# tensor4all/tensor4all-rs

Hardware: AMD Instinct MI355X
Metric: TCI2 full-sweep GF/s (d=30, chi=256 fp64) (higher is better)
Workload: dtype f64

## Files before the change

### tensor4all-rs_amd/csrc/kernels.hpp

```cpp
#pragma once

#include <hip/hip_runtime.h>

#include <cstddef>
#include <cstdint>

#include "../../include/t4a_testfunctions.h"

namespace t4a {

struct RrluWorkspace;

struct RrluPlan {
    int W = 1;
    int T = 256;
    int cpw = 0;
    int Mld = 0;
    size_t lds_bytes = 0;
};

RrluPlan rrlu_make_plan(int M, int N, int num_cus);

struct RrluArgs {
    const double* A;
// ... 150 lines not shown
    unsigned long long* h_block;
    int block_u64;
    const int* dims;
    int dims_swap;
    const int* rowmap;
    XcdSpecArgs spec;
    int ts_u64;
};
bool rrlu_xcd_make_plan(int M, int N, RrluXcdPlan* out, bool any_size = false, int max_w = 32, bool allow_big = false);
size_t rrlu_xcd_keys_bytes(const RrluXcdPlan& plan);
size_t rrlu_xcd_cols_bytes(const RrluXcdPlan& plan, int M);
struct RrluXcdGroupArgs {
    RrluXcdArgs p[8];
};
void rrlu_xcd2_launch(const RrluXcdPlan& plan, const RrluXcdArgs& args, hipStream_t stream);
void rrlu_xcd2m_launch(const RrluXcdPlan& plan, const RrluXcdArgs& args, hipStream_t stream);
void rrlu_xcd2_group_launch(const RrluXcdPlan& plan, const RrluXcdGroupArgs& args, bool tie_row_major, hipStream_t stream);
bool rrlu_wg_make_plan(int M, int N, RrluXcdPlan* out, int spec_blocks = 0);
void rrlu_wg_launch(const RrluXcdPlan& plan, const RrluXcdArgs& args, hipStream_t stream);
void rrlu_wg_group_launch(const RrluXcdPlan& plan, const RrluXcdGroupArgs& args, bool tie_row_major, hipStream_t stream);
bool rrlu_w1_make_plan(int M, int N, RrluXcdPlan* out, int spec_blocks = 0);
void rrlu_w1_launch(const RrluXcdPlan& plan, const RrluXcdArgs& args, hipStream_t stream);
void rrlu_w1_group_launch(const RrluXcdPlan& plan, const RrluXcdGroupArgs& args, bool tie_row_major, hipStream_t stream);

void pi_eval_launch(const FnDevice& fn, const uint64_t* rowacc, int M, const uint64_t* colacc, int N, double* out,
                    int ld, bool transpose_out, unsigned long long* max_abs_bits, hipStream_t stream);
struct PiJob {
    const uint64_t* rowacc;
    const uint64_t* colacc;
    double* out;
    unsigned long long* max_abs_bits;
    int M, N, ld, pad_;
};
void pi_eval_batched_launch(const FnDevice& fn, const PiJob* d_jobs, int n_jobs, int max_M, int max_N, hipStream_t stream);
struct PackJob {
    const double* src;
    double* core;
    const int* info;
    int ld, L, S, R, last, pad_;
};
struct LuProblem;
constexpr int FILL_SMALL_MAX_N = 32, FILL_SMALL_MAX_RHS = 64;
void fill_small_launch(const FnDevice& fn, const PiJob* d_pis, const LuProblem* d_lups, const PackJob* d_packs, int n_jobs, int last_site,
                       hipStream_t stream);
void stage_copy_launch(const uint64_t* pinned_src, uint64_t* dst, size_t count, hipStream_t stream);
void absmax_launch(const double* data, size_t count, unsigned long long* max_abs_bits, hipStream_t stream);

constexpr int CHAIN_MAX_SET = 1024;
struct ChainTab {
    uint64_t* code;
    uint64_t* acc;
    int* cnt;
};
struct ChainCommon {
    ChainTab I, J, HI, HJ;
    ChainTab mI, mJ;
    int cap, K;
    const uint64_t* w;
    int total;
    const int* ldim;
    const int* woff;
    int forward, use_extras;
    int one_site;
    uint64_t* ind_code;
    uint64_t* ind_acc;
    int* ind_cnt;
    int ind_cap;
// ... 105 lines not shown
                               double* left, double* right, hipStream_t stream);
void transpose_launch(const double* in, int rows, int cols, int ldi, double* out, int ldo, hipStream_t stream);

struct TrsmProblem {
    const double* T; int ldt; int n;
    double* B; int ldb; int nrhs;
    int lower; int unit_diag;
    const int* skip_flag;
};
void trsm_left_batched_launch(const TrsmProblem* d_problems, int n_problems, int max_n, int max_nrhs, hipStream_t stream);

struct LuProblem {
    double* A; int lda; int n;
    int* piv;
    int* info;
    double* B; int ldb; int nrhs;
    const unsigned long long* pmax_bits;
};
void lu_batched_launch(const LuProblem* d_problems, int n_problems, int max_n, hipStream_t stream);
inline TrsmProblem lu_trsm_problem(const LuProblem& lp, bool lower, const int* skip_flag = nullptr)
{
    TrsmProblem t{};
    t.T = lp.A;
    t.ldt = lp.lda;
    t.n = lp.n;
    t.B = lp.B;
    t.ldb = lp.ldb;
    t.nrhs = lp.nrhs;
    t.lower = t.unit_diag = lower ? 1 : 0;
    t.skip_flag = skip_flag;
    return t;
}
constexpr int LU_MAX_PANEL_STEPS = 128;
bool lu_forward_blocked_launch(const LuProblem* d_problems, int n_problems, int max_n, int max_nrhs, hipStream_t stream, int avoid_xcc = -1,
                               unsigned* tickets = nullptr);
bool lu_solve_blocked_launch(const LuProblem* d_problems, int n_problems, int max_n, int max_nrhs, hipStream_t stream, int avoid_xcc = -1,
                             unsigned* tickets = nullptr);

void gather_launch(const double* in, int ldi, const int* rows, int nrows, const int* cols, int ncols, double* out,
                   int ldo, hipStream_t stream);
void scatter_rows_launch(const double* in, int ldi, const int* rows, int nrows, int ncols, double* out, int ldo,
                         hipStream_t stream);
void scatter_cols_launch(const double* in, int ldi, int nrows, const int* cols, int ncols, double* out, int ldo,
                         hipStream_t stream);
void fill_launch(double* p, size_t count, double value, hipStream_t stream);
void seq_matmul_launch(const double* A, int lda, const double* B, int ldb, double* C, int ldc, size_t M, size_t N, size_t K,
                       hipStream_t stream);
void set_identity_launch(double* p, int m, int n, int ld, hipStream_t stream);

struct TtCoreDesc { const double* data; int l, d, r; };
void tt_evaluate_launch(const TtCoreDesc* d_cores, int n_sites, int max_bond, const uint32_t* d_idx, int n_pts,
                        double* d_out, hipStream_t stream);


void core_reshape_launch(const double* in, int L, int S, int R, int mode, double* out, hipStream_t stream);
constexpr int PERMUTE_MAX_RANK = 16;
void permute_launch(const double* in, const size_t* dims, const size_t* perm, int rank, double* out, hipStream_t stream);
void tt_sum_launch(const TtCoreDesc* d_cores, int n_sites, int max_bond, double* d_out, hipStream_t stream);
void tt_norm2_step_launch(const TtCoreDesc& core, const double* d_cur, bool first, double* d_nxt, hipStream_t stream);
void tt_env_left_launch(const TtCoreDesc* d_cores, int split, int max_bond, const uint32_t* d_idx, int n_items,
                        double* d_out, int ld, hipStream_t stream);
void tt_env_right_launch(const TtCoreDesc* d_cores, int n_sites, int split, int max_bond, const uint32_t* d_idx,
                         int n_items, double* d_out, int ld, hipStream_t stream);
void tt_env_dot_launch(const double* d_left, const double* d_right, int len, int ld, const uint32_t* d_il,
                       const uint32_t* d_ir, size_t n_pts, double* d_out, hipStream_t stream);

struct MpoSiteJob {
    const double* A;
    const double* B;
// ... 100 lines not shown
```

### tensor4all-rs_amd/csrc/kernels_dense.hip

```cpp
#include "kernels.hpp"

#include <algorithm>
#include <atomic>
#include <map>
#include <mutex>
#include <utility>
#include "common.hpp"

#include <cstdlib>

namespace t4a {

namespace {

typedef double double4_t __attribute__((ext_vector_type(4)));

constexpr int GBM = 64, GBK = 32, GPAD = 4;

template <int BN>
__global__ void __launch_bounds__(256) gemm_kernel(GemmDesc d)
{
    extern __shared__ __attribute__((aligned(16))) char gemm_smem[];
    typedef double TileA[GBK][GBM + GPAD];
    typedef double TileB[GBK][BN + GPAD];
// ... 615 lines not shown
                for (int c = 0; c < NB; ++c) a[r][c] = U[c];
            }
            if (i == prow) {
#pragma unroll
                for (int c = 0; c < NB; ++c) a[r][c] = V[c];
            }
        }
    }
    const double piv = U[J];
    if (piv == 0.0 || piv != piv) return;
#pragma unroll
    for (int r = 0; r < RP; ++r) {
        const int i = tid + 256 * r;
        if (i > J && i < m) {
            const double l = a[r][J] / piv;
            a[r][J] = l;
#pragma unroll
            for (int c = J + 1; c < NB; ++c) {
                const double prod = l * U[c];
                a[r][c] = a[r][c] - prod;
            }
        }
    }
}

template <int NB, int RP, int... Js>
__device__ __forceinline__ void lu_panel_columns(double (&a)[RP][NB], const PanelShared& sh, const LuProblem& pr, int kb, int m, int w, int tid,
                                                 int& first_bad, std::integer_sequence<int, Js...>)
{
    (lu_panel_column<NB, RP, Js>(a, sh, pr, kb, m, w, tid, first_bad), ...);
}

template <int NB, int RP>
__global__ void __launch_bounds__(256) lu_panel_kernel(const LuProblem* problems, int kb)
{
    __shared__ double U[2 * NB], V[2 * NB];
    __shared__ double red_v[8];
    __shared__ int red_i[8];
    const LuProblem pr = problems[blockIdx.x];
    const int n = pr.n;
    const int tid = threadIdx.x;
    if (kb == 0) {
        if (pr.pmax_bits) {
            const double pmax = __longlong_as_double((long long)*pr.pmax_bits);
            if (pmax < 2.220446049250313e-16) {
                if (tid == 0) pr.info[0] = -1;
                return;
            }
        }
        if (tid == 0) pr.info[0] = 0;
    } else if (pr.info[0] == -1) {
        return;
    }
    if (kb >= n) return;
    const int m = n - kb, w = (n - kb) < NB ? (n - kb) : NB;
    double* A = pr.A;
    const int lda = pr.lda;
    double a[RP][NB];
#pragma unroll
    for (int r = 0; r < RP; ++r) {
        const int i = tid + 256 * r;
#pragma unroll
        for (int c = 0; c < NB; ++c) a[r][c] = (i < m && c < w) ? A[(size_t)(kb + c) * lda + kb + i] : 0.0;
    }
    int first_bad = 0;
    PanelShared sh{U, V, red_v, red_i};
    lu_panel_columns<NB, RP>(a, sh, pr, kb, m, w, tid, first_bad, std::make_integer_sequence<int, NB>{});
    if (tid == 0 && first_bad != 0 && pr.info[0] == 0) pr.info[0] = first_bad;
#pragma unroll
    for (int r = 0; r < RP; ++r) {
        const int i = tid + 256 * r;
#pragma unroll
        for (int c = 0; c < NB; ++c)
            if (i < m && c < w) A[(size_t)(kb + c) * lda + kb + i] = a[r][c];
    }
}

__global__ void __launch_bounds__(256) lu_update_kernel(const LuProblem* problems, int kb, int nb, int tiles, int n_problems, int avoid_xcc,
                                                        unsigned* ticket, int a_only)
{
    extern __shared__ __attribute__((aligned(16))) char smem_raw[];
    __shared__ int s_item;
    if (avoid_xcc >= 0) {
        unsigned xcc;
        asm volatile("s_getreg_b32 %0, hwreg(HW_REG_XCC_ID)" : "=s"(xcc));
        if ((int)(xcc & 0xF) == avoid_xcc) return;
    }
    const int total_items = tiles * n_problems;
    bool first = true;
    for (;;) {
    __syncthreads();
    if (threadIdx.x == 0) s_item = ticket ? (int)atomicAdd(ticket, 1u) : (first ? (int)blockIdx.x : total_items);
    __syncthreads();
    first = false;
    const int item = s_item;
    if (item >= total_items) break;
    const LuProblem pr = problems[item / tiles];
    const int n = pr.n;
    if (kb >= n || pr.info[0] == -1) continue;
    const int ta = (n + nb - 1) / nb;
    const int nrhs = pr.B ? pr.nrhs : 0;
    const int t = item % tiles;
    const bool in_a = t < ta;
    const int c0 = in_a ? t * nb : (t - ta) * nb;
    if (!in_a && (a_only || c0 >= nrhs)) continue;
    if (in_a && c0 == kb) continue;
    const int m = n - kb, w = (n - kb) < nb ? (n - kb) : nb;
    const int lim = in_a ? n : nrhs;
    const int tc = (lim - c0) < nb ? (lim - c0) : nb;
    const bool left = in_a && c0 < kb;
    const int tid = threadIdx.x, T = blockDim.x;
    const int ldp = m | 1;
    double* L = (double*)smem_raw;
    double* Tt = L + (size_t)ldp * nb;
    auto gcol = [&](int c) -> double* {
        return in_a ? pr.A + (size_t)(c0 + c) * pr.lda + kb : pr.B + (size_t)(c0 + c) * pr.ldb + kb;
    };
    {
        const double* const tbase = in_a ? pr.A + (size_t)c0 * pr.lda + kb : pr.B + (size_t)c0 * pr.ldb + kb;
// ... 85 lines not shown
        double* g = gcol(c);
        for (int i = tid; i < m; i += T) g[i] = Tt[(size_t)c * ldp + i];
    }
    }
}


constexpr int SVB = 16;
constexpr int SV_MAXS = 8;
template <int Q> __device__ __forceinline__ double quad_bcast_f64(double v)
{
    constexpr int ctrl = Q | (Q << 2) | (Q << 4) | (Q << 6);
    const long long b = __double_as_longlong(v);
    const int lo = __builtin_amdgcn_update_dpp(0, (int)(b & 0xFFFFFFFFll), ctrl, 0xF, 0xF, true);
    const int hi = __builtin_amdgcn_update_dpp(0, (int)(b >> 32), ctrl, 0xF, 0xF, true);
    return __longlong_as_double(((long long)hi << 32) | (unsigned int)lo);
}
template <int KK, bool LOWER> __device__ __forceinline__ void solve_block_step(double (&b)[4], const double (&dr)[SVB][4], const double (&rdr)[SVB], int g)
{
    constexpr int go = KK >> 2, to = KK & 3;
    double xk = quad_bcast_f64<go>(b[to]);
    if (!LOWER) xk = xk * rdr[KK];
    if (g == go) b[to] = xk;
#pragma unroll
    for (int t = 0; t < 4; ++t) b[t] = __builtin_fma(-dr[KK][t], xk, b[t]);
}
template <bool LOWER, int... KKs>
__device__ __forceinline__ void solve_block_steps(double (&b)[4], const double (&dr)[SVB][4], const double (&rdr)[SVB], int g, std::integer_sequence<int, KKs...>)
{
    if constexpr (LOWER) (solve_block_step<KKs, true>(b, dr, rdr, g), ...);
    else (solve_block_step<SVB - 1 - KKs, false>(b, dr, rdr, g), ...);
}

__global__ void __launch_bounds__(256) __attribute__((amdgpu_waves_per_eu(1, 1))) lu_solve_kernel(const LuProblem* problems, int cw, int n_problems, int chunks, int avoid_xcc, unsigned* ticket)
{
    extern __shared__ __attribute__((aligned(16))) char smem_raw[];
    __shared__ int s_item;
    if (avoid_xcc >= 0) {
        unsigned xcc;
        asm volatile("s_getreg_b32 %0, hwreg(HW_REG_XCC_ID)" : "=s"(xcc));
        if ((int)(xcc & 0xF) == avoid_xcc) return;
    }
    const int tid = threadIdx.x;
    const int lane = tid & 63, wave = tid >> 6;
    const int lr = lane & 15, lk = lane >> 4;
    const int cl = lane >> 2, g = lane & 3;
    const int total_items = chunks * n_problems;
    bool first = true;
    for (;;) {
        __syncthreads();
        if (tid == 0) s_item = ticket ? (int)atomicAdd(ticket, 1u) : (first ? (int)blockIdx.x : total_items);
        __syncthreads();
        first = false;
        const int item = s_item;
        if (item >= total_items) break;
        const LuProblem pr = problems[item / chunks];
        const int n = pr.n;
        const int c0 = (item % chunks) * cw;
        if (n <= 0 || !pr.B || c0 >= pr.nrhs || pr.info[0] == -1) continue;
        const int cwr = (pr.nrhs - c0) < cw ? (pr.nrhs - c0) : cw;
        const int ld = n | 1;
        double* Bs = reinterpret_cast<double*>(smem_raw);
        double* D = Bs + (size_t)ld * cw + ((ld * cw) & 1);
        double* rd = D + SVB * SVB;
        unsigned short* perm_s = reinterpret_cast<unsigned short*>(rd + SVB);
        unsigned short* piv_s = perm_s + ((n + 3) & ~3);
        typedef const double __attribute__((address_space(1)))* gcptr;
        typedef double __attribute__((address_space(1)))* gptr;
        const gcptr T = (gcptr)pr.A;
        const gptr Bg = (gptr)pr.B;
        const int ldt = pr.lda;
        {
            const int G = (n + 31) / 32;
            unsigned short* gs = reinterpret_cast<unsigned short*>(smem_raw);
// ... 401 lines not shown
            (void)hipFuncSetAttribute(reinterpret_cast<const void*>(&trsm_left_mfma_kernel), hipFuncAttributeMaxDynamicSharedMemorySize,
                                      160 * 1024);
            attr2 = true;
        }
        int cw = 32;
        const size_t per_col = (size_t)(max_n | 1) * 8;
        while (cw > 16 && (per_col * cw + (TRB + 1) * TRB * 8 > 150 * 1024 || (long long)n_problems * max_nrhs / cw < 1024)) cw -= 16;
        const size_t lds = per_col * cw + (size_t)(TRB + 1) * TRB * 8;
        if (lds <= 160 * 1024) {
            dim3 grid((max_nrhs + cw - 1) / cw, n_problems);
            hipLaunchKernelGGL(trsm_left_mfma_kernel, grid, dim3(256), lds, stream, d_problems, cw);
            return;
        }
    }
    int cw = (int)((128 * 1024) / ((size_t)max_n * 8));
    if (cw > 32) cw = 32;
    const long long total_cols = (long long)n_problems * max_nrhs;
    while (cw > 4 && total_cols / cw < 2048) cw /= 2;
    if (cw < 1) cw = 1;
    const size_t lds = (size_t)max_n * cw * 8;
    if (lds > 160 * 1024)
        throw Error(T4A_GPU_NOT_IMPLEMENTED, "triangular solve: systems with more than 20480 rows are not supported");
    dim3 grid((max_nrhs + cw - 1) / cw, n_problems);
    hipLaunchKernelGGL(trsm_left_kernel, grid, dim3(256), lds, stream, d_problems, cw);
}

void lu_batched_launch(const LuProblem* d_problems, int n_problems, int max_n, hipStream_t stream)
{
    if (n_problems <= 0) return;
    int T = max_n >= 128 ? 1024 : (max_n >= 32 ? 256 : 64);
    hipLaunchKernelGGL(lu_kernel, dim3(n_problems), dim3(T), 0, stream, d_problems);
}

bool lu_forward_blocked_launch(const LuProblem* d_problems, int n_problems, int max_n, int max_nrhs, hipStream_t stream, int avoid_xcc,
                               unsigned* tickets)
{
    if (n_problems <= 0 || max_n <= 0) return true;
    int nb;
    if (max_n <= 256) nb = 32;
    else if (max_n <= 512) nb = 16;
    else if (max_n <= 1024) nb = 8;
    else return false;
    static std::atomic<bool> attr_set{false};
    if (!attr_set) {
        (void)hipFuncSetAttribute(reinterpret_cast<const void*>(&lu_update_kernel),
                                  hipFuncAttributeMaxDynamicSharedMemorySize, 144 * 1024);
        (void)hipGetLastError();
        attr_set = true;
    }
    const int ldp = max_n | 1;
    const size_t lds_update = (size_t)ldp * nb * 8 * 2;
    const int tiles = (max_n + nb - 1) / nb + (max_nrhs + nb - 1) / nb + 1;
    for (int kb = 0; kb < max_n; kb += nb) {
        if (nb == 32) hipLaunchKernelGGL((lu_panel_kernel<32, 1>), dim3(n_problems), dim3(256), 0, stream, d_problems, kb);
        else if (nb == 16) hipLaunchKernelGGL((lu_panel_kernel<16, 2>), dim3(n_problems), dim3(256), 0, stream, d_problems, kb);
        else hipLaunchKernelGGL((lu_panel_kernel<8, 4>), dim3(n_problems), dim3(256), 0, stream, d_problems, kb);
        const int items = tiles * n_problems;
        unsigned* tk = tickets ? tickets + kb / nb : nullptr;
        const int grid = tk ? items + items / 7 + 8 : items;
        hipLaunchKernelGGL(lu_update_kernel, dim3(grid), dim3(256), lds_update, stream, d_problems, kb, nb, tiles, n_problems,
                           tk ? avoid_xcc : -1, tk, 0);
    }
    return true;
}

bool lu_solve_blocked_launch(const LuProblem* d_problems, int n_problems, int max_n, int max_nrhs, hipStream_t stream, int avoid_xcc,
                             unsigned* tickets)
{
    if (n_problems <= 0 || max_n <= 0) return true;
    if (max_n < 32 || max_n > 16 * 4 * SV_MAXS || max_nrhs < 16) return false;
    int nb;
    if (max_n <= 256) nb = 32;
    else nb = 16;
    static std::once_flag attr_once;
    std::call_once(attr_once, [] {
        (void)hipFuncSetAttribute(reinterpret_cast<const void*>(&lu_update_kernel), hipFuncAttributeMaxDynamicSharedMemorySize, 144 * 1024);
        (void)hipFuncSetAttribute(reinterpret_cast<const void*>(&lu_solve_kernel), hipFuncAttributeMaxDynamicSharedMemorySize, 160 * 1024);
        (void)hipGetLastError();
    });
    const int ldp = max_n | 1;
    const size_t lds_update = (size_t)ldp * nb * 8 * 2;
    const int tiles = (max_n + nb - 1) / nb;
    for (int kb = 0; kb < max_n; kb += nb) {
        if (nb == 32) hipLaunchKernelGGL((lu_panel_kernel<32, 1>), dim3(n_problems), dim3(256), 0, stream, d_problems, kb);
        else hipLaunchKernelGGL((lu_panel_kernel<16, 2>), dim3(n_problems), dim3(256), 0, stream, d_problems, kb);
        const int items = tiles * n_problems;
        unsigned* tk = tickets ? tickets + kb / nb : nullptr;
        const int grid = tk ? items + items / 7 + 8 : items;
        hipLaunchKernelGGL(lu_update_kernel, dim3(grid), dim3(256), lds_update, stream, d_problems, kb, nb, tiles, n_problems,
                           tk ? avoid_xcc : -1, tk, 1);
    }
    const size_t extra = (size_t)SVB * (SVB + 1) * 8 + SVB * 8 + 2 * (size_t)((max_n + 3) & ~3) * 2 + 64;
    int cw = 64;
    while (cw > 16 && (size_t)(max_n | 1) * cw * 8 + extra > 156 * 1024) cw -= 16;
    if (cw == 48) cw = 32;
    while (cw > 16 && max_nrhs <= cw / 2) cw /= 2;
    const size_t lds = (size_t)(max_n | 1) * cw * 8 + extra;
    const int chunks = (max_nrhs + cw - 1) / cw;
    const int items = chunks * n_problems;
    unsigned* tk = tickets ? tickets + (LU_MAX_PANEL_STEPS - 1) : nullptr;
    const int grid = tk ? items + items / 7 + 8 : items;
    hipLaunchKernelGGL(lu_solve_kernel, dim3(grid), dim3(256), lds, stream, d_problems, cw, n_problems, chunks, tk ? avoid_xcc : -1, tk);
    return true;
}

void tt_evaluate_launch(const TtCoreDesc* d_cores, int n_sites, int max_bond, const uint32_t* d_idx, int n_pts,
                        double* d_out, hipStream_t stream)
{
    if (n_pts <= 0) return;
    int blocks = n_pts < 4096 ? n_pts : 4096;
    const size_t lds = (size_t)2 * (max_bond > 0 ? max_bond : 1) * 8;
    hipLaunchKernelGGL(tt_eval_kernel, dim3(blocks), dim3(256), lds, stream, d_cores, n_sites, max_bond, d_idx, n_pts,
                       d_out);
}

}
```

### tensor4all-rs_amd/csrc/kernels_pi.hip

```cpp
#include "kernels.hpp"

namespace t4a {

namespace {

__device__ __forceinline__ void wave_absmax_commit(double av, unsigned long long* max_abs_bits)
{
#pragma unroll
    for (int off = 32; off >= 1; off >>= 1) {
        const double o = __shfl_xor(av, off);
        if (o > av) av = o;
    }
    if ((threadIdx.x & 63) == 0 && av > 0.0 && max_abs_bits)
        atomicMax(max_abs_bits, (unsigned long long)__double_as_longlong(av));
}

__global__ void __launch_bounds__(256) pi_eval_kernel(FnDevice fn, const uint64_t* __restrict__ rowacc, int M,
                                                      const uint64_t* __restrict__ colacc, int N,
                                                      double* __restrict__ out, int ld, int transpose_out,
                                                      unsigned long long* max_abs_bits)
{
    double av = 0.0;
    const int i = blockIdx.x * blockDim.x + threadIdx.x;
    uint64_t racc[T4A_FN_MAX_ACC] = {0, 0, 0, 0};
    if (i < M)
        for (int k = 0; k < fn.n_acc; ++k) racc[k] = rowacc[(size_t)i * fn.n_acc + k];
    for (int j = blockIdx.y; j < N; j += gridDim.y) {
        if (i < M) {
            uint64_t acc[T4A_FN_MAX_ACC] = {0, 0, 0, 0};
            for (int k = 0; k < fn.n_acc; ++k) acc[k] = racc[k] + colacc[(size_t)j * fn.n_acc + k];
            const double v = t4a_fn_value(fn.fid, acc, fn.params);
            if (transpose_out)
                out[(size_t)i * ld + j] = v;
            else
                out[(size_t)j * ld + i] = v;
            const double a = sqrt(v * v);
            if (a > av) av = a;
        }
    }
    wave_absmax_commit(av, max_abs_bits);
}

__global__ void __launch_bounds__(256) pi_eval_batched_kernel(FnDevice fn, const PiJob* __restrict__ jobs)
{
    const PiJob jb = jobs[blockIdx.z];
    double av = 0.0;
    const int i = blockIdx.x * blockDim.x + threadIdx.x;
    if (blockIdx.x * (int)blockDim.x >= jb.M) return;
    uint64_t racc[T4A_FN_MAX_ACC] = {0, 0, 0, 0};
    if (i < jb.M)
        for (int k = 0; k < fn.n_acc; ++k) racc[k] = jb.rowacc[(size_t)i * fn.n_acc + k];
    for (int j = blockIdx.y; j < jb.N; j += gridDim.y) {
        if (i < jb.M) {
            uint64_t acc[T4A_FN_MAX_ACC] = {0, 0, 0, 0};
            for (int k = 0; k < fn.n_acc; ++k) acc[k] = racc[k] + jb.colacc[(size_t)j * fn.n_acc + k];
            const double v = t4a_fn_value(fn.fid, acc, fn.params);
            jb.out[(size_t)j * jb.ld + i] = v;
            const double a = sqrt(v * v);
            if (a > av) av = a;
        }
    }
    wave_absmax_commit(av, jb.max_abs_bits);
}

__global__ void __launch_bounds__(256) absmax_kernel(const double* __restrict__ data, size_t count,
                                                     unsigned long long* max_abs_bits)
{
    double av = 0.0;
    for (size_t i = (size_t)blockIdx.x * blockDim.x + threadIdx.x; i < count; i += (size_t)gridDim.x * blockDim.x) {
        const double v = data[i];
        const double a = sqrt(v * v);
        if (a > av) av = a;
    }
    wave_absmax_commit(av, max_abs_bits);
}

__global__ void __launch_bounds__(256) stage_copy_kernel(const uint64_t* __restrict__ src, uint64_t* __restrict__ dst, size_t count)
{
    for (size_t i = (size_t)blockIdx.x * blockDim.x + threadIdx.x; i < count; i += (size_t)gridDim.x * blockDim.x) dst[i] = src[i];
}

}

void stage_copy_launch(const uint64_t* pinned_src, uint64_t* dst, size_t count, hipStream_t stream)
{
    if (count == 0) return;
    size_t blocks = (count + 255) / 256;
    if (blocks > 64) blocks = 64;
    hipLaunchKernelGGL(stage_copy_kernel, dim3((unsigned)blocks), dim3(256), 0, stream, pinned_src, dst, count);
}

void pi_eval_launch(const FnDevice& fn, const uint64_t* rowacc, int M, const uint64_t* colacc, int N, double* out,
                    int ld, bool transpose_out, unsigned long long* max_abs_bits, hipStream_t stream)
{
    if (M <= 0 || N <= 0) return;
    dim3 block(256);
    int gy = N < 2048 ? N : 2048;
    dim3 grid((M + 255) / 256, gy);
    hipLaunchKernelGGL(pi_eval_kernel, grid, block, 0, stream, fn, rowacc, M, colacc, N, out, ld,
                       transpose_out ? 1 : 0, max_abs_bits);
}

void pi_eval_batched_launch(const FnDevice& fn, const PiJob* d_jobs, int n_jobs, int max_M, int max_N, hipStream_t stream)
{
    if (n_jobs <= 0 || max_M <= 0 || max_N <= 0) return;
    const int gy = max_N < 512 ? max_N : 512;
    dim3 grid((max_M + 255) / 256, gy, n_jobs);
    hipLaunchKernelGGL(pi_eval_batched_kernel, grid, dim3(256), 0, stream, fn, d_jobs);
}

namespace {

struct FillSmallArgs {
    FnDevice fn;
    const PiJob* pis;
    const LuProblem* lups;
    const PackJob* packs;
    int n_jobs, last_site;
};

__global__ void __launch_bounds__(256) fill_small_kernel(FillSmallArgs a)
{
    __shared__ double As[FILL_SMALL_MAX_N * FILL_SMALL_MAX_N];
    __shared__ double Bs[FILL_SMALL_MAX_N * FILL_SMALL_MAX_RHS];
    __shared__ double red_v[4];
    __shared__ int red_i[4];
    __shared__ int piv_s, info_s;
    __shared__ double pivval_s;
    const int k = blockIdx.x, tid = threadIdx.x, T = blockDim.x, lane = tid & 63, wave = tid >> 6;
    if (k >= a.n_jobs) return;
    const bool last = a.last_site && k == a.n_jobs - 1;
    const int K = a.fn.n_acc;
    double pmax = 0.0;
    for (int q = 0; q < (last ? 1 : 2); ++q) {
        const PiJob jb = a.pis[2 * k + q];
        double* const dst = q == 0 ? Bs : As;
        double av = 0.0;
        for (int e = tid; e < jb.M * jb.N; e += T) {
            const int i = e % jb.M, j = e / jb.M;
            uint64_t acc[T4A_FN_MAX_ACC] = {0, 0, 0, 0};
            for (int c = 0; c < K; ++c) acc[c] = jb.rowacc[(size_t)i * K + c] + jb.colacc[(size_t)j * K + c];
// ... 156 lines not shown
```

### tensor4all-rs_amd/csrc/tci2.hip

```cpp
#include "tci2.hpp"

#include <thread>

#include <exception>

#include <algorithm>
#include <atomic>
#include <chrono>
#include <cmath>
#include <cstdlib>
#include <string>
#include <unordered_set>

namespace t4a {

extern thread_local double g_chain_wait_seconds;

namespace {

__global__ void __launch_bounds__(256) pack_left_core_kernel(const double* __restrict__ mat, int ldm, int mrows,
                                                             int mcols, double* __restrict__ core, int L, int S, int R)
{
    const size_t total = (size_t)L * S * R;
    for (size_t e = (size_t)blockIdx.x * blockDim.x + threadIdx.x; e < total; e += (size_t)gridDim.x * blockDim.x) {
// ... 914 lines not shown
    fill_last_sig_ = sig;
    ++fill_stats_[0];
    if (!done)
        for (auto& f : ops) f();
    if (fill_timed_) T4A_HIP(hipEventRecord(ev_fill_.b, st));
}

void Tci2::fill_wait()
{
    if (import_inflight_) {
        import_inflight_ = false;
        T4A_HIP(hipStreamSynchronize(import_stream_));
    }
    if (!fill_inflight_) return;
    fill_inflight_ = false;
    T4A_HIP(hipStreamSynchronize(fill_stream_));
    T4A_HIP(hipGetLastError());
    if (eng.prof.enabled && fill_timed_) {
        float ms = 0.f;
        T4A_HIP(hipEventElapsedTime(&ms, ev_fill_.a, ev_fill_.b));
        eng.prof.v[4] += ms;
        eng.prof.v[5] += 1.0;
    }
    fill_timed_ = false;
    for (size_t k = 0; k < fill_solved_sites_.size(); ++k)
        if (h_fillinfo_.get()[fill_solved_sites_[k]] > 0) {
            const size_t site = fill_solved_sites_[k];
            fill_solved_sites_.clear();
            throw Error(T4A_GPU_INTERNAL_ERROR, "one-site interpolation solve failed: singular pivot matrix at site " +
                                                    std::to_string(site));
        }
    fill_solved_sites_.clear();
}

void Tci2::fill_site_tensors_impl(bool async)
{
    fn_.require("tci2");
    const bool trust_cache = fill_cache_trusted_;
    fill_cache_trusted_ = false;
    static const bool host_prof_fill = std::getenv("T4A_HOST_PROFILE") != nullptr;
    const auto hpf_t0 = std::chrono::steady_clock::now();
    static double hpf_sec[10] = {0, 0, 0, 0, 0, 0, 0, 0, 0, 0};
    auto hpf_mark = [&](int k, std::chrono::steady_clock::time_point& t) {
        if (!host_prof_fill) return;
        const auto now = std::chrono::steady_clock::now();
        hpf_sec[k] += std::chrono::duration<double, std::micro>(now - t).count();
        t = now;
    };
    auto hpf_t = hpf_t0;
    if (!trust_cache) invalidate_fill_cache();
    if (!fn_.builtin()) sync_digits();
    fill_wait();
    if (!fill_stream_) fill_stream_ = pool::stream_get(2);
    const bool builtin = fn_.builtin();
    static const bool sync_fill = std::getenv("T4A_SYNC_FILL") != nullptr;
    if (!builtin || sync_fill) async = false;
    std::vector<std::function<void()>> ops;
    std::vector<uint64_t> sig;
    auto dev = [&](std::function<void()> f) { ops.push_back(std::move(f)); };
    auto sg = [&](uint64_t v) { sig.push_back(v); };
    const bool no_main_sync = fill_no_main_sync_ && fn_.builtin();
    fill_no_main_sync_ = false;
    if (!no_main_sync) T4A_HIP(hipStreamSynchronize(eng.stream()));
    hipStream_t st = fill_stream_;
    struct SiteJob {
        size_t b;
// ... 25 lines not shown
                dev([=]() { fill_launch(ptr, cnt, 0.0, st); });
            }
            continue;
        }
        SiteJob j;
        j.b = b;
        j.ni = ni;
        j.nj = nj;
        j.last = (b == n_ - 1);
        j.np = j.last ? 0 : i_set[b + 1].count;
        if (!j.last && j.np != nj)
            throw Error(T4A_GPU_INTERNAL_ERROR, "one-site interpolation solve failed: pivot matrix at bond " +
                                                    std::to_string(b) + " is not square (" + std::to_string(j.np) + " x " +
                                                    std::to_string(nj) + ")");
        j.offA = totA;
        j.offB = totB;
        j.accJ = j.accK = j.accI = 0;
        totA += j.last ? 0 : nj * j.np;
        totB += nj * ni;
        jobs.push_back(j);
    }
    hpf_mark(0, hpf_t);
    if (jobs.empty()) {
        for (auto& f : ops) f();
        T4A_HIP(hipStreamSynchronize(st));
        return;
    }
    if (!builtin) {
        for (auto& f : ops) f();
        ops.clear();
    }
    d_fillA_.reserve(std::max<size_t>(totA, 1));
    d_fillB_.reserve(totB);
    const size_t fm_words = n_ + (n_ + 1) / 2 + (LU_MAX_PANEL_STEPS + 1) / 2;
    d_fillmax_.reserve(fm_words);
    unsigned long long* d_max = d_fillmax_.get();
    int* d_info = reinterpret_cast<int*>(d_fillmax_.get() + n_);
    unsigned* d_tickets = reinterpret_cast<unsigned*>(d_fillmax_.get() + n_ + (n_ + 1) / 2);
    const int avoid_xcc = (no_main_sync && !xcd_disabled()) ? eng.xcc() : -1;
    h_fillinfo_.reserve(n_);
    {
        unsigned long long* ptr = d_fillmax_.get();
        const size_t bytes = fm_words * sizeof(unsigned long long);
        fill_timed_ = eng.prof.enabled;
        sg((uint64_t)(uintptr_t)ptr);
        sg((uint64_t)bytes);
        dev([=]() { T4A_HIP(hipMemsetAsync(ptr, 0, bytes, st)); });
        if (!builtin) {
            if (fill_timed_) T4A_HIP(hipEventRecord(ev_fill_.a, st));
            for (auto& f : ops) f();
            ops.clear();
            T4A_HIP(hipStreamSynchronize(st));
        }
    }

    for (const SiteJob& j : jobs) {
        const size_t left_dim = (j.b == 0) ? 1 : i_set[j.b].count;
        const size_t S = local_dims[j.b];
        DevCore& c = cores[j.b];
        c.l = left_dim;
        c.s = S;
        c.r = j.last ? 1 : j.np;
        c.buf.reserve(std::max<size_t>(c.size(), 1));
    }

    std::vector<LuProblem> lups;
    std::vector<TrsmProblem> trl, tru;
    std::vector<PackJob> packs;
    size_t piv_total = 0;
    for (const SiteJob& j : jobs)
        if (!j.last) piv_total += j.np;
    d_fillpiv_.reserve(std::max<size_t>(piv_total, 1));
// ... 115 lines not shown
                q.out = d_fillA_.get() + j.offA;
                q.max_abs_bits = d_max + j.b;
                pis.push_back(q);
            }
        }
        for (const PiJob& q : pis) {
            max_M = std::max(max_M, q.M);
            max_N = std::max(max_N, q.N);
        }
        std::memcpy(hb + off_pi, pis.data(), pis.size() * sizeof(PiJob));
        if (np_) {
            std::memcpy(hb + off_lu, lups.data(), bytes_lu);
            std::memcpy(hb + off_tr, trl.data(), np_ * sizeof(TrsmProblem));
            std::memcpy(hb + off_tr + np_ * sizeof(TrsmProblem), tru.data(), np_ * sizeof(TrsmProblem));
        }
        std::memcpy(hb + off_pk, packs.data(), bytes_pk);
        hpf_mark(7, hpf_t);
        {
            const FnDevice fn = fn_.dev;
            const PiJob* dj = reinterpret_cast<const PiJob*>(db + off_pi);
            const int npi = (int)pis.size();
            sg((uint64_t)(uintptr_t)db);
            sg((uint64_t)(uintptr_t)hb);
            sg((uint64_t)total_bytes);
            sg((uint64_t)npi);
            sg(((uint64_t)(uint32_t)max_M << 32) | (uint32_t)max_N);
            sg((uint64_t)fn.fid * 16 + (uint64_t)fn.n_acc);
            for (int q = 0; q < T4A_FN_MAX_PARAMS; ++q) {
                uint64_t bits;
                std::memcpy(&bits, &fn.params[q], sizeof(bits));
                sg(bits);
            }
            sg((uint64_t)small_fill);
            const bool small = small_fill;
            dev([=]() {
                T4A_HIP(hipMemcpyAsync(db, hb, total_bytes, hipMemcpyHostToDevice, st));
                if (!small) pi_eval_batched_launch(fn, dj, npi, max_M, max_N, st);
            });
        }
        d_lups = reinterpret_cast<const LuProblem*>(db + off_lu);
        d_trs = reinterpret_cast<const TrsmProblem*>(db + off_tr);
        d_packs = reinterpret_cast<const PackJob*>(db + off_pk);
        d_pis = reinterpret_cast<const PiJob*>(db + off_pi);
    } else {
        for (const SiteJob& j : jobs) {
            IndexSet ik = kronecker_i(j.b);
            const IndexSet& jb = j_set[j.b];
            if (j.last) {
                eval_matrix(ik, 0, jb, ik.width, d_fillB_.get() + j.offB, nullptr);
            } else {
                eval_matrix(jb, j.b + 1, ik, 0, d_fillB_.get() + j.offB, nullptr);
                eval_matrix(jb, j.b + 1, i_set[j.b + 1], 0, d_fillA_.get() + j.offA, d_max + j.b);
            }
        }
        T4A_HIP(hipStreamSynchronize(eng.stream()));
        acc_used_ = 0;
        const size_t off_tr = up8(bytes_lu), off_pk = up8(off_tr + bytes_tr), total_bytes = up8(off_pk + bytes_pk);
        h_fillacc_.reserve(total_bytes / 8 + 1);
        d_fillacc_.reserve(total_bytes / 8 + 1);
        char* hb = reinterpret_cast<char*>(h_fillacc_.get());
        char* db = reinterpret_cast<char*>(d_fillacc_.get());
        if (np_) {
            std::memcpy(hb, lups.data(), bytes_lu);
            std::memcpy(hb + off_tr, trl.data(), np_ * sizeof(TrsmProblem));
            std::memcpy(hb + off_tr + np_ * sizeof(TrsmProblem), tru.data(), np_ * sizeof(TrsmProblem));
        }
        std::memcpy(hb + off_pk, packs.data(), bytes_pk);
        T4A_HIP(hipMemcpyAsync(db, hb, total_bytes, hipMemcpyHostToDevice, st));
        d_lups = reinterpret_cast<const LuProblem*>(db);
        d_trs = reinterpret_cast<const TrsmProblem*>(db + off_tr);
        d_packs = reinterpret_cast<const PackJob*>(db + off_pk);
    }

    {
        const int npr = (int)np_;
        const unsigned gx = blocks_for(max_core) > 64 ? 64 : blocks_for(max_core), gy = (unsigned)packs.size();
        int* hinfo = h_fillinfo_.get();
        const size_t info_bytes = n_ * sizeof(int);
        sg((uint64_t)npr);
        sg((uint64_t)(int64_t)avoid_xcc);
        sg(((uint64_t)(uint32_t)max_n << 32) | (uint32_t)max_nrhs);
        sg(((uint64_t)gx << 32) | gy);
        sg((uint64_t)(uintptr_t)d_lups);
        sg((uint64_t)(uintptr_t)d_trs);
        sg((uint64_t)(uintptr_t)d_packs);
        sg((uint64_t)(uintptr_t)d_info);
        sg((uint64_t)(uintptr_t)hinfo);
        const FnDevice fn = fn_.dev;
        const int n_site_jobs = (int)jobs.size(), last_site = jobs.back().last ? 1 : 0;
        const bool small = small_fill;
        sg((uint64_t)(uintptr_t)d_pis);
        sg(((uint64_t)n_site_jobs << 1) | (uint64_t)last_site);
        dev([=]() {
            if (small) {
                fill_small_launch(fn, d_pis, d_lups, d_packs, n_site_jobs, last_site, st);
                T4A_HIP(hipMemcpyAsync(hinfo, d_info, info_bytes, hipMemcpyDeviceToHost, st));
                return;
            }
            if (npr) {
                if (!lu_solve_blocked_launch(d_lups, npr, max_n, max_nrhs, st, avoid_xcc, d_tickets)) {
                    if (!lu_forward_blocked_launch(d_lups, npr, max_n, max_nrhs, st, avoid_xcc, d_tickets)) {
                        lu_batched_launch(d_lups, npr, max_n, st);
                        trsm_left_batched_launch(d_trs, npr, max_n, max_nrhs, st);
                    }
                    trsm_left_batched_launch(d_trs + npr, npr, max_n, max_nrhs, st);
                }
            }
            hipLaunchKernelGGL(pack_fill_batched_kernel, dim3(gx, gy), dim3(256), 0, st, d_packs);
            T4A_HIP(hipMemcpyAsync(hinfo, d_info, info_bytes, hipMemcpyDeviceToHost, st));
        });
    }
    hpf_mark(3, hpf_t);
    eng.prof.v[10] += flops;
    if (!builtin) {
        for (auto& f : ops) f();
        if (fill_timed_) T4A_HIP(hipEventRecord(ev_fill_.b, st));
        fill_inflight_ = true;
    } else {
        issue_fill_ops(ops, sig);
        fill_inflight_ = true;
    }
    if (host_prof_fill) {
        static double acc_ms = 0;
        static long calls = 0;
        acc_ms += std::chrono::duration<double, std::milli>(std::chrono::steady_clock::now() - hpf_t0).count();
        hpf_mark(4, hpf_t);
        if (++calls % 20 == 0)
            std::fprintf(stderr, "[host profile] fill_site_tensors host part %.1f us per call (wait+jobs %.1f, descriptors %.1f, "
                                 "accumulators %.1f, staging %.1f, issue %.1f)\n",
                         1e3 * acc_ms / calls, hpf_sec[0] / calls, hpf_sec[1] / calls, hpf_sec[2] / calls, hpf_sec[3] / calls,
                         hpf_sec[4] / calls);
        if (calls % 20 == 0)
            std::fprintf(stderr, "[host profile]   staging in detail: reserve %.1f, accumulator copy %.1f, job tables %.1f us per call\n",
                         hpf_sec[5] / calls, hpf_sec[6] / calls, hpf_sec[7] / calls);
// ... 253 lines not shown
    r.small_complete = false;
    if (small_engine_run(r) && r.small_complete) return;
    if (fn_.builtin() && options.max_bond_dim != 0 && options.max_bond_dim <= 1024) {
        const size_t chi = options.max_bond_dim;
        std::vector<size_t> lb(n_ + 1, 1), rb(n_ + 1, 1);
        for (size_t b = 0; b < n_; ++b) lb[b + 1] = std::min(chi, lb[b] * local_dims[b]);
        for (size_t b = n_; b-- > 0;) rb[b] = std::min(chi, rb[b + 1] * local_dims[b]);
        auto bond = [&](size_t b) { return std::min(lb[b], rb[b]); };
        size_t totA = 0, totB = 0, tot_cores = 0;
        for (size_t b = 0; b < n_; ++b) {
            if (shard_world > 1 && (b % shard_world) != shard_rank) continue;
            const size_t l = bond(b), rr = bond(b + 1);
            tot_cores += l * local_dims[b] * rr;
            totA += rr * rr;
            totB += rr * l * local_dims[b];
        }
        const bool presize = (tot_cores + totA + totB) * sizeof(double) <= ((size_t)1 << 30);
        for (size_t b = 0; presize && b < n_; ++b) {
            if (shard_world > 1 && (b % shard_world) != shard_rank) continue;
            cores[b].buf.reserve(std::max<size_t>(bond(b) * local_dims[b] * bond(b + 1), 1));
        }
        if (presize) {
        d_fillA_.reserve(std::max<size_t>(totA, 1));
        d_fillB_.reserve(std::max<size_t>(totB, 1));
        d_fillpiv_.reserve(std::max<size_t>(n_ * chi, 1));
        size_t acc_words = 0;
        for (size_t b = 0; b < n_; ++b) {
            if (shard_world > 1 && (b % shard_world) != shard_rank) continue;
            acc_words += chi * (2 + local_dims[b]) * (size_t)fn_.dev.n_acc;
        }
        const size_t desc_bytes = n_ * (2 * sizeof(PiJob) + sizeof(LuProblem) + 2 * sizeof(TrsmProblem) + 64) + 256;
        h_fillacc_.reserve(acc_words + desc_bytes / 8 + 64);
        d_fillacc_.reserve(acc_words + desc_bytes / 8 + 64);
        d_fillmax_.reserve(n_ + (n_ + 1) / 2 + (LU_MAX_PANEL_STEPS + 1) / 2);
        h_fillinfo_.reserve(n_);
        }
    }
}

bool Tci2::opt_iter_start(OptRun& r, bool defer_launch)
{
    const TCI2Options& options = r.options;
    if (r.done || r.iter >= options.max_iter) return false;
    const size_t iter = r.iter;
    (void)iter;
        r.norm = (options.normalize_error && max_sample_value > 0.0) ? max_sample_value : 1.0;
        r.abs_tol = options.tolerance * r.norm;
        bool is_forward = true;
        if (options.sweep_strategy == 1) is_forward = false;
        else if (options.sweep_strategy == 2) is_forward = (iter % 2 == 0);

        long ext_idx = (!options.strictly_nested && !history.empty()) ? (long)history.size() - 1 : -1;
        {
            OptSeg seg_(0);
            HistEntry cur;
            cur.serial = ++chain_.hist_serial;
            if (chain_.digits_stale) {
                cur.digits_valid = false;
                cur.cap = chain_.cap;
                cur.is.resize(n_);
                cur.js.resize(n_);
                for (size_t p = 0; p < n_; ++p) {
                    cur.is[p].width = i_set[p].width;
                    cur.is[p].count = i_set[p].count;
                    cur.js[p].width = j_set[p].width;
                    cur.js[p].count = j_set[p].count;
                }
// ... 296 lines not shown
```

Measured before the change: 306.5.

## Steer fill kernels away from all XCDs busy with concurrent multi-XCD rrLU

```diff
diff --git a/tensor4all-rs_amd/csrc/kernels.hpp b/tensor4all-rs_amd/csrc/kernels.hpp
--- a/tensor4all-rs_amd/csrc/kernels.hpp
+++ b/tensor4all-rs_amd/csrc/kernels.hpp
@@ -206,7 +206,9 @@
     unsigned long long* max_abs_bits;
     int M, N, ld, pad_;
 };
-void pi_eval_batched_launch(const FnDevice& fn, const PiJob* d_jobs, int n_jobs, int max_M, int max_N, hipStream_t stream);
+constexpr int PI_MAX_ITEMS = 4096;
+void pi_eval_batched_launch(const FnDevice& fn, const PiJob* d_jobs, int n_jobs, int max_M, int max_N, hipStream_t stream,
+                            unsigned avoid_mask = 0, unsigned* ticket = nullptr);
 struct PackJob {
     const double* src;
     double* core;
@@ -378,9 +380,10 @@
     return t;
 }
 constexpr int LU_MAX_PANEL_STEPS = 128;
-bool lu_forward_blocked_launch(const LuProblem* d_problems, int n_problems, int max_n, int max_nrhs, hipStream_t stream, int avoid_xcc = -1,
+constexpr int LU_TICKET_WORDS = 2 * LU_MAX_PANEL_STEPS;
+bool lu_forward_blocked_launch(const LuProblem* d_problems, int n_problems, int max_n, int max_nrhs, hipStream_t stream, unsigned avoid_mask = 0,
                                unsigned* tickets = nullptr);
-bool lu_solve_blocked_launch(const LuProblem* d_problems, int n_problems, int max_n, int max_nrhs, hipStream_t stream, int avoid_xcc = -1,
+bool lu_solve_blocked_launch(const LuProblem* d_problems, int n_problems, int max_n, int max_nrhs, hipStream_t stream, unsigned avoid_mask = 0,
                              unsigned* tickets = nullptr);
 
 void gather_launch(const double* in, int ldi, const int* rows, int nrows, const int* cols, int ncols, double* out,
diff --git a/tensor4all-rs_amd/csrc/kernels_dense.hip b/tensor4all-rs_amd/csrc/kernels_dense.hip
--- a/tensor4all-rs_amd/csrc/kernels_dense.hip
+++ b/tensor4all-rs_amd/csrc/kernels_dense.hip
@@ -671,12 +671,8 @@
 }
 
 template <int NB, int RP>
-__global__ void __launch_bounds__(256) lu_panel_kernel(const LuProblem* problems, int kb)
-{
-    __shared__ double U[2 * NB], V[2 * NB];
-    __shared__ double red_v[8];
-    __shared__ int red_i[8];
-    const LuProblem pr = problems[blockIdx.x];
+__device__ __forceinline__ void lu_panel_problem(const LuProblem& pr, int kb, const PanelShared& sh)
+{
     const int n = pr.n;
     const int tid = threadIdx.x;
     if (kb == 0) {
@@ -703,7 +699,6 @@
         for (int c = 0; c < NB; ++c) a[r][c] = (i < m && c < w) ? A[(size_t)(kb + c) * lda + kb + i] : 0.0;
     }
     int first_bad = 0;
-    PanelShared sh{U, V, red_v, red_i};
     lu_panel_columns<NB, RP>(a, sh, pr, kb, m, w, tid, first_bad, std::make_integer_sequence<int, NB>{});
     if (tid == 0 && first_bad != 0 && pr.info[0] == 0) pr.info[0] = first_bad;
 #pragma unroll
@@ -715,15 +710,42 @@
     }
 }
 
-__global__ void __launch_bounds__(256) lu_update_kernel(const LuProblem* problems, int kb, int nb, int tiles, int n_problems, int avoid_xcc,
+template <int NB, int RP>
+__global__ void __launch_bounds__(256) __attribute__((amdgpu_waves_per_eu(5))) lu_panel_kernel(const LuProblem* problems, int kb, int n_problems, unsigned avoid_mask, unsigned* ticket)
+{
+    __shared__ double U[2 * NB], V[2 * NB];
+    __shared__ double red_v[8];
+    __shared__ int red_i[8];
+    __shared__ int s_item;
+    PanelShared sh{U, V, red_v, red_i};
+    if (!ticket) {
+        lu_panel_problem<NB, RP>(problems[blockIdx.x], kb, sh);
+        return;
+    }
+    {
+        unsigned xcc;
+        asm volatile("s_getreg_b32 %0, hwreg(HW_REG_XCC_ID)" : "=s"(xcc));
+        if ((avoid_mask >> (xcc & 0xF)) & 1u) return;
+    }
+    for (;;) {
+        __syncthreads();
+        if (threadIdx.x == 0) s_item = (int)atomicAdd(ticket, 1u);
+        __syncthreads();
+        const int item = __builtin_amdgcn_readfirstlane(s_item);
+        if (item >= n_problems) break;
+        lu_panel_problem<NB, RP>(problems[item], kb, sh);
+    }
+}
+
+__global__ void __launch_bounds__(256) lu_update_kernel(const LuProblem* problems, int kb, int nb, int tiles, int n_problems, unsigned avoid_mask,
                                                         unsigned* ticket, int a_only)
 {
     extern __shared__ __attribute__((aligned(16))) char smem_raw[];
     __shared__ int s_item;
-    if (avoid_xcc >= 0) {
+    if (avoid_mask) {
         unsigned xcc;
         asm volatile("s_getreg_b32 %0, hwreg(HW_REG_XCC_ID)" : "=s"(xcc));
-        if ((int)(xcc & 0xF) == avoid_xcc) return;
+        if ((avoid_mask >> (xcc & 0xF)) & 1u) return;
     }
     const int total_items = tiles * n_problems;
     bool first = true;
@@ -875,14 +897,14 @@
     else (solve_block_step<SVB - 1 - KKs, false>(b, dr, rdr, g), ...);
 }
 
-__global__ void __launch_bounds__(256) __attribute__((amdgpu_waves_per_eu(1, 1))) lu_solve_kernel(const LuProblem* problems, int cw, int n_problems, int chunks, int avoid_xcc, unsigned* ticket)
+__global__ void __launch_bounds__(256) __attribute__((amdgpu_waves_per_eu(1, 1))) lu_solve_kernel(const LuProblem* problems, int cw, int n_problems, int chunks, unsigned avoid_mask, unsigned* ticket)
 {
     extern __shared__ __attribute__((aligned(16))) char smem_raw[];
     __shared__ int s_item;
-    if (avoid_xcc >= 0) {
+    if (avoid_mask) {
         unsigned xcc;
         asm volatile("s_getreg_b32 %0, hwreg(HW_REG_XCC_ID)" : "=s"(xcc));
-        if ((int)(xcc & 0xF) == avoid_xcc) return;
+        if ((avoid_mask >> (xcc & 0xF)) & 1u) return;
     }
     const int tid = threadIdx.x;
     const int lane = tid & 63, wave = tid >> 6;
@@ -1350,7 +1372,7 @@
     hipLaunchKernelGGL(lu_kernel, dim3(n_problems), dim3(T), 0, stream, d_problems);
 }
 
-bool lu_forward_blocked_launch(const LuProblem* d_problems, int n_problems, int max_n, int max_nrhs, hipStream_t stream, int avoid_xcc,
+bool lu_forward_blocked_launch(const LuProblem* d_problems, int n_problems, int max_n, int max_nrhs, hipStream_t stream, unsigned avoid_mask,
                                unsigned* tickets)
 {
     if (n_problems <= 0 || max_n <= 0) return true;
@@ -1370,19 +1392,21 @@
     const size_t lds_update = (size_t)ldp * nb * 8 * 2;
     const int tiles = (max_n + nb - 1) / nb + (max_nrhs + nb - 1) / nb + 1;
     for (int kb = 0; kb < max_n; kb += nb) {
-        if (nb == 32) hipLaunchKernelGGL((lu_panel_kernel<32, 1>), dim3(n_problems), dim3(256), 0, stream, d_problems, kb);
-        else if (nb == 16) hipLaunchKernelGGL((lu_panel_kernel<16, 2>), dim3(n_problems), dim3(256), 0, stream, d_problems, kb);
-        else hipLaunchKernelGGL((lu_panel_kernel<8, 4>), dim3(n_problems), dim3(256), 0, stream, d_problems, kb);
+        unsigned* ptk = (tickets && avoid_mask) ? tickets + LU_MAX_PANEL_STEPS + kb / nb : nullptr;
+        const int pgrid = ptk ? n_problems + n_problems / 7 + 8 : n_problems;
+        if (nb == 32) hipLaunchKernelGGL((lu_panel_kernel<32, 1>), dim3(pgrid), dim3(256), 0, stream, d_problems, kb, n_problems, avoid_mask, ptk);
+        else if (nb == 16) hipLaunchKernelGGL((lu_panel_kernel<16, 2>), dim3(pgrid), dim3(256), 0, stream, d_problems, kb, n_problems, avoid_mask, ptk);
+        else hipLaunchKernelGGL((lu_panel_kernel<8, 4>), dim3(pgrid), dim3(256), 0, stream, d_problems, kb, n_problems, avoid_mask, ptk);
         const int items = tiles * n_problems;
         unsigned* tk = tickets ? tickets + kb / nb : nullptr;
         const int grid = tk ? items + items / 7 + 8 : items;
         hipLaunchKernelGGL(lu_update_kernel, dim3(grid), dim3(256), lds_update, stream, d_problems, kb, nb, tiles, n_problems,
-                           tk ? avoid_xcc : -1, tk, 0);
+                           tk ? avoid_mask : 0u, tk, 0);
     }
     return true;
 }
 
-bool lu_solve_blocked_launch(const LuProblem* d_problems, int n_problems, int max_n, int max_nrhs, hipStream_t stream, int avoid_xcc,
+bool lu_solve_blocked_launch(const LuProblem* d_problems, int n_problems, int max_n, int max_nrhs, hipStream_t stream, unsigned avoid_mask,
                              unsigned* tickets)
 {
     if (n_problems <= 0 || max_n <= 0) return true;
@@ -1400,13 +1424,15 @@
     const size_t lds_update = (size_t)ldp * nb * 8 * 2;
     const int tiles = (max_n + nb - 1) / nb;
     for (int kb = 0; kb < max_n; kb += nb) {
-        if (nb == 32) hipLaunchKernelGGL((lu_panel_kernel<32, 1>), dim3(n_problems), dim3(256), 0, stream, d_problems, kb);
-        else hipLaunchKernelGGL((lu_panel_kernel<16, 2>), dim3(n_problems), dim3(256), 0, stream, d_problems, kb);
+        unsigned* ptk = (tickets && avoid_mask) ? tickets + LU_MAX_PANEL_STEPS + kb / nb : nullptr;
+        const int pgrid = ptk ? n_problems + n_problems / 7 + 8 : n_problems;
+        if (nb == 32) hipLaunchKernelGGL((lu_panel_kernel<32, 1>), dim3(pgrid), dim3(256), 0, stream, d_problems, kb, n_problems, avoid_mask, ptk);
+        else hipLaunchKernelGGL((lu_panel_kernel<16, 2>), dim3(pgrid), dim3(256), 0, stream, d_problems, kb, n_problems, avoid_mask, ptk);
         const int items = tiles * n_problems;
         unsigned* tk = tickets ? tickets + kb / nb : nullptr;
         const int grid = tk ? items + items / 7 + 8 : items;
         hipLaunchKernelGGL(lu_update_kernel, dim3(grid), dim3(256), lds_update, stream, d_problems, kb, nb, tiles, n_problems,
-                           tk ? avoid_xcc : -1, tk, 1);
+                           tk ? avoid_mask : 0u, tk, 1);
     }
     const size_t extra = (size_t)SVB * (SVB + 1) * 8 + SVB * 8 + 2 * (size_t)((max_n + 3) & ~3) * 2 + 64;
     int cw = 64;
@@ -1418,7 +1444,7 @@
     const int items = chunks * n_problems;
     unsigned* tk = tickets ? tickets + (LU_MAX_PANEL_STEPS - 1) : nullptr;
     const int grid = tk ? items + items / 7 + 8 : items;
-    hipLaunchKernelGGL(lu_solve_kernel, dim3(grid), dim3(256), lds, stream, d_problems, cw, n_problems, chunks, tk ? avoid_xcc : -1, tk);
+    hipLaunchKernelGGL(lu_solve_kernel, dim3(grid), dim3(256), lds, stream, d_problems, cw, n_problems, chunks, tk ? avoid_mask : 0u, tk);
     return true;
 }
 
diff --git a/tensor4all-rs_amd/csrc/kernels_pi.hip b/tensor4all-rs_amd/csrc/kernels_pi.hip
--- a/tensor4all-rs_amd/csrc/kernels_pi.hip
+++ b/tensor4all-rs_amd/csrc/kernels_pi.hip
@@ -41,16 +41,14 @@
     wave_absmax_commit(av, max_abs_bits);
 }
 
-__global__ void __launch_bounds__(256) pi_eval_batched_kernel(FnDevice fn, const PiJob* __restrict__ jobs)
-{
-    const PiJob jb = jobs[blockIdx.z];
+__device__ __forceinline__ void pi_eval_job_columns(const FnDevice& fn, const PiJob& jb, int row0, int j0, int j1, int jstep)
+{
     double av = 0.0;
-    const int i = blockIdx.x * blockDim.x + threadIdx.x;
-    if (blockIdx.x * (int)blockDim.x >= jb.M) return;
+    const int i = row0 + (int)threadIdx.x;
     uint64_t racc[T4A_FN_MAX_ACC] = {0, 0, 0, 0};
     if (i < jb.M)
         for (int k = 0; k < fn.n_acc; ++k) racc[k] = jb.rowacc[(size_t)i * fn.n_acc + k];
-    for (int j = blockIdx.y; j < jb.N; j += gridDim.y) {
+    for (int j = j0; j < j1; j += jstep) {
         if (i < jb.M) {
             uint64_t acc[T4A_FN_MAX_ACC] = {0, 0, 0, 0};
             for (int k = 0; k < fn.n_acc; ++k) acc[k] = racc[k] + jb.colacc[(size_t)j * fn.n_acc + k];
@@ -63,6 +61,39 @@
     wave_absmax_commit(av, jb.max_abs_bits);
 }
 
+__global__ void __launch_bounds__(256) pi_eval_batched_kernel(FnDevice fn, const PiJob* __restrict__ jobs, unsigned avoid_mask,
+                                                              unsigned* ticket, int row_tiles, int col_blocks, int col_block, int n_jobs)
+{
+    if (!ticket) {
+        const PiJob jb = jobs[blockIdx.z];
+        if (blockIdx.x * (int)blockDim.x >= jb.M) return;
+        pi_eval_job_columns(fn, jb, blockIdx.x * blockDim.x, blockIdx.y, jb.N, gridDim.y);
+        return;
+    }
+    __shared__ int s_item;
+    {
+        unsigned xcc;
+        asm volatile("s_getreg_b32 %0, hwreg(HW_REG_XCC_ID)" : "=s"(xcc));
+        if ((avoid_mask >> (xcc & 0xF)) & 1u) return;
+    }
+    const int per_job = row_tiles * col_blocks, total_items = per_job * n_jobs;
+    if (threadIdx.x == 0) s_item = (int)atomicAdd(ticket, 1u);
+    __syncthreads();
+    int item = __builtin_amdgcn_readfirstlane(s_item);
+    while (item < total_items) {
+        unsigned next = 0;
+        if (threadIdx.x == 0) next = atomicAdd(ticket, 1u);
+        const PiJob jb = jobs[item / per_job];
+        const int r = item % per_job;
+        const int row0 = (r / col_blocks) * 256, c0 = (r % col_blocks) * col_block;
+        if (row0 < jb.M && c0 < jb.N) pi_eval_job_columns(fn, jb, row0, c0, (c0 + col_block) < jb.N ? (c0 + col_block) : jb.N, 1);
+        __syncthreads();
+        if (threadIdx.x == 0) s_item = (int)next;
+        __syncthreads();
+        item = __builtin_amdgcn_readfirstlane(s_item);
+    }
+}
+
 __global__ void __launch_bounds__(256) absmax_kernel(const double* __restrict__ data, size_t count,
                                                      unsigned long long* max_abs_bits)
 {
@@ -101,12 +132,23 @@
                        transpose_out ? 1 : 0, max_abs_bits);
 }
 
-void pi_eval_batched_launch(const FnDevice& fn, const PiJob* d_jobs, int n_jobs, int max_M, int max_N, hipStream_t stream)
+void pi_eval_batched_launch(const FnDevice& fn, const PiJob* d_jobs, int n_jobs, int max_M, int max_N, hipStream_t stream,
+                            unsigned avoid_mask, unsigned* ticket)
 {
     if (n_jobs <= 0 || max_M <= 0 || max_N <= 0) return;
+    const int row_tiles = (max_M + 255) / 256;
+    if (avoid_mask && ticket) {
+        int col_block = 4;
+        while ((long long)n_jobs * row_tiles * ((max_N + col_block - 1) / col_block) > PI_MAX_ITEMS) col_block *= 2;
+        const int col_blocks = (max_N + col_block - 1) / col_block;
+        const int items = n_jobs * row_tiles * col_blocks;
+        hipLaunchKernelGGL(pi_eval_batched_kernel, dim3(items + items / 7 + 8), dim3(256), 0, stream, fn, d_jobs, avoid_mask, ticket,
+                           row_tiles, col_blocks, col_block, n_jobs);
+        return;
+    }
     const int gy = max_N < 512 ? max_N : 512;
-    dim3 grid((max_M + 255) / 256, gy, n_jobs);
-    hipLaunchKernelGGL(pi_eval_batched_kernel, grid, dim3(256), 0, stream, fn, d_jobs);
+    dim3 grid(row_tiles, gy, n_jobs);
+    hipLaunchKernelGGL(pi_eval_batched_kernel, grid, dim3(256), 0, stream, fn, d_jobs, 0u, (unsigned*)nullptr, 0, 0, 0, n_jobs);
 }
 
 namespace {
diff --git a/tensor4all-rs_amd/csrc/tci2.hip b/tensor4all-rs_amd/csrc/tci2.hip
--- a/tensor4all-rs_amd/csrc/tci2.hip
+++ b/tensor4all-rs_amd/csrc/tci2.hip
@@ -970,6 +970,8 @@
         }
     fill_solved_sites_.clear();
 }
+
+static size_t fill_scratch_words(size_t n) { return n + (n + 1) / 2 + (LU_TICKET_WORDS + 1 + 1) / 2; }
 
 void Tci2::fill_site_tensors_impl(bool async)
 {
@@ -1061,12 +1063,20 @@
     }
     d_fillA_.reserve(std::max<size_t>(totA, 1));
     d_fillB_.reserve(totB);
-    const size_t fm_words = n_ + (n_ + 1) / 2 + (LU_MAX_PANEL_STEPS + 1) / 2;
+    const size_t fm_words = fill_scratch_words(n_);
     d_fillmax_.reserve(fm_words);
     unsigned long long* d_max = d_fillmax_.get();
     int* d_info = reinterpret_cast<int*>(d_fillmax_.get() + n_);
     unsigned* d_tickets = reinterpret_cast<unsigned*>(d_fillmax_.get() + n_ + (n_ + 1) / 2);
-    const int avoid_xcc = (no_main_sync && !xcd_disabled()) ? eng.xcc() : -1;
+    unsigned* d_pi_ticket = d_tickets + LU_TICKET_WORDS;
+    unsigned avoid_mask = 0;
+    if (no_main_sync && !xcd_disabled()) {
+        int k_max = 1;
+        if (chain_.inflight)
+            for (const RrluRoute& pl : chain_.plans)
+                if (pl.kind == RrluKind::MultiXcd) k_max = std::max(k_max, pl.xcd.K);
+        for (int k = 0; k < std::min(k_max, 4); ++k) avoid_mask |= 1u << ((eng.xcc() + k) & 7);
+    }
     h_fillinfo_.reserve(n_);
     {
         unsigned long long* ptr = d_fillmax_.get();
@@ -1248,10 +1258,12 @@
                 sg(bits);
             }
             sg((uint64_t)small_fill);
+            sg((uint64_t)avoid_mask);
+            sg((uint64_t)(uintptr_t)d_pi_ticket);
             const bool small = small_fill;
             dev([=]() {
                 T4A_HIP(hipMemcpyAsync(db, hb, total_bytes, hipMemcpyHostToDevice, st));
-                if (!small) pi_eval_batched_launch(fn, dj, npi, max_M, max_N, st);
+                if (!small) pi_eval_batched_launch(fn, dj, npi, max_M, max_N, st, avoid_mask, d_pi_ticket);
             });
         }
         d_lups = reinterpret_cast<const LuProblem*>(db + off_lu);
@@ -1294,7 +1306,8 @@
         int* hinfo = h_fillinfo_.get();
         const size_t info_bytes = n_ * sizeof(int);
         sg((uint64_t)npr);
-        sg((uint64_t)(int64_t)avoid_xcc);
+        sg((uint64_t)avoid_mask);
+        sg((uint64_t)(uintptr_t)d_tickets);
         sg(((uint64_t)(uint32_t)max_n << 32) | (uint32_t)max_nrhs);
         sg(((uint64_t)gx << 32) | gy);
         sg((uint64_t)(uintptr_t)d_lups);
@@ -1314,8 +1327,8 @@
                 return;
             }
             if (npr) {
-                if (!lu_solve_blocked_launch(d_lups, npr, max_n, max_nrhs, st, avoid_xcc, d_tickets)) {
-                    if (!lu_forward_blocked_launch(d_lups, npr, max_n, max_nrhs, st, avoid_xcc, d_tickets)) {
+                if (!lu_solve_blocked_launch(d_lups, npr, max_n, max_nrhs, st, avoid_mask, d_tickets)) {
+                    if (!lu_forward_blocked_launch(d_lups, npr, max_n, max_nrhs, st, avoid_mask, d_tickets)) {
                         lu_batched_launch(d_lups, npr, max_n, st);
                         trsm_left_batched_launch(d_trs, npr, max_n, max_nrhs, st);
                     }
@@ -1635,7 +1648,7 @@
         const size_t desc_bytes = n_ * (2 * sizeof(PiJob) + sizeof(LuProblem) + 2 * sizeof(TrsmProblem) + 64) + 256;
         h_fillacc_.reserve(acc_words + desc_bytes / 8 + 64);
         d_fillacc_.reserve(acc_words + desc_bytes / 8 + 64);
-        d_fillmax_.reserve(n_ + (n_ + 1) / 2 + (LU_MAX_PANEL_STEPS + 1) / 2);
+        d_fillmax_.reserve(fill_scratch_words(n_));
         h_fillinfo_.reserve(n_);
         }
     }
```

After: 307.5, median of 6. About the same (+0.3%).
